# nv-tlabs/NKSR

Hardware: AMD Instinct MI355X
Metric: reconstructed points/sec (solve+mesh) (higher is better)
Workload: dtype f32

## Files before the change

### include/nksr_hip.h

```cpp
#ifndef NKSR_HIP_H
#define NKSR_HIP_H
#include <stddef.h>
#include <stdint.h>

#ifdef __cplusplus
extern "C" {
#endif

#define NKSR_MAX_DEPTH 6
#define NKSR_OK 0
#define NKSR_ERR_ARG (-1)
#define NKSR_ERR_HIP (-2)
#define NKSR_ERR_CAPACITY (-3)

const char* nksr_last_error(void);
int nksr_version(void);

typedef struct {
    int32_t n;
    int32_t offset;
    const int64_t* keys;
    const int32_t* ijk;
    const int32_t* nbr;
    const int64_t* hkeys;
// ... 239 lines not shown
int nksr_edge_seam_flags(const nksr_chunk_grid_t* grid, const int64_t* vkey, const int8_t* axis, int64_t n, int32_t cells_per_voxel, float w0,
                         const int32_t* owner, int32_t rank, uint8_t* flags_out, void* stream);
int nksr_points_owner_flags(const nksr_chunk_grid_t* grid, const float* xyz, int64_t n, float reach, const int32_t* owner, int32_t rank,
                            uint8_t* flags_out, void* stream);
int nksr_halo_band_flags(const int64_t* keys, const int32_t* ijk, int64_t n, const int64_t* klo, int32_t nchunk, const float* shift,
                         const float* tlo, const float* thi, float w, int32_t* seg_out, int32_t* flags_out, void* stream);

int nksr_knn_pca_normals(const float* xyz_sorted, int64_t n, const int32_t* start, const int32_t* end,
                         const int64_t* hkeys, const int32_t* hvals, int32_t hcap, float cell, float inv_cell, int k,
                         int max_ring, float* normal_out, float* radius2_out, int32_t* valid_out,
                         int32_t* todo_work ,
                         void* stream);
#define NKSR_KNN_LEVELS 12
typedef struct {
    const float* xyz_sorted;
    const int32_t* start[NKSR_KNN_LEVELS];
    const int32_t* end[NKSR_KNN_LEVELS];
    const int32_t* child[NKSR_KNN_LEVELS];
    const uint8_t* cmask[NKSR_KNN_LEVELS];
    const int64_t* hkeys[NKSR_KNN_LEVELS];
    const int32_t* hvals[NKSR_KNN_LEVELS];
    int32_t hcap[NKSR_KNN_LEVELS];
    int32_t levels, leaf;
    float cell, inv_cell;
} nksr_knn_pyramid_t;
int nksr_knn_pyramid_level(const int64_t* child_keys, int32_t n_child, const int32_t* child_start, const int32_t* child_end,
                           const int64_t* keys, int32_t n, int32_t* child_out, uint8_t* cmask_out, int32_t* start_out, int32_t* end_out,
                           void* stream);
int nksr_sdf_from_points_pyramid(const nksr_knn_pyramid_t* pyramid, const float* normal_sorted, const float* ref_std_sorted, const float* query,
                                 int64_t nq, int k, int max_ring, float stdv, int imls, float* sdf_out, float* grad_out, int32_t* valid_out,
                                 void* stream);
int nksr_knn_mean_dist_pyramid(const nksr_knn_pyramid_t* pyramid, int64_t n, int k, int max_ring, float* out, int32_t* valid_out, void* stream);
int nksr_sdf_from_points(const float* xyz_sorted, const float* normal_sorted, const float* ref_std_sorted, const int32_t* start,
                         const int32_t* end, const int64_t* hkeys, const int32_t* hvals, int32_t hcap, float cell, float inv_cell,
                         const float* query, int64_t nq, int k, int max_ring, float stdv, int imls, float* sdf_out, float* grad_out,
                         int32_t* valid_out, void* stream);
int nksr_knn_mean_dist(const float* xyz_sorted, int64_t n, const int32_t* start, const int32_t* end, const int64_t* hkeys,
                       const int32_t* hvals, int32_t hcap, float cell, float inv_cell, int k, int max_ring, float* out,
                       int32_t* valid_out, void* stream);
int nksr_nearest_index(const float* xyz_sorted, const int32_t* start, const int32_t* end, const int64_t* hkeys,
                       const int32_t* hvals, int32_t hcap, float cell, float inv_cell, const float* query, int64_t nq,
                       int max_ring, int32_t* index_out, void* stream);
int nksr_knn_query_pyramid(const nksr_knn_pyramid_t* pyramid, int64_t n_ref, const float* query, int64_t nq, int k, int exclude_self,
                           const int32_t* self_index, int max_ring, int32_t* idx_out, float* dist2_out, int32_t* valid_out, void* stream);
int nksr_radius_count(const float* xyz_sorted, int64_t n_ref, const int32_t* start, const int32_t* end, const int64_t* hkeys,
                      const int32_t* hvals, int32_t hcap, float cell, float inv_cell, const float* query, int64_t nq, float radius,
                      int32_t cap, int exclude_self, const int32_t* self_index, int32_t* count_out, void* stream);

#define NKSR_ICP_BLOCK 256
#define NKSR_ICP_FIELDS 32
#define NKSR_ICP_COUNT 0
#define NKSR_ICP_D2 1
#define NKSR_ICP_PT_P 2
#define NKSR_ICP_PT_Q 5
#define NKSR_ICP_PT_PQ 8
#define NKSR_ICP_PL_JJ 2
#define NKSR_ICP_PL_JR 23
#define NKSR_ICP_PL_RR 29
int nksr_icp_accumulate(const float* xyz_sorted, int64_t n_ref, const int32_t* start, const int32_t* end, const int64_t* hkeys,
                        const int32_t* hvals, int32_t hcap, float cell, float inv_cell, const int64_t* perm, const float* normal_sorted,
                        const float* source, int64_t n_src, const double* transform, const double* centre, float radius, int method,
                        int64_t* corr_out, double* partials_out, void* stream);
int nksr_icp_reduce(const double* partials, int64_t nrows, double* sums_out, void* stream);

#define NKSR_VOXEL_REDUCE_MAX_C 16
int nksr_voxel_reduce(const int32_t* order, int64_t n, const int32_t* start, const int32_t* end, int64_t n_vox, const float* xyz,
                      const float* attr, int C, int group, float* mean_xyz_out, float* mean_attr_out, int32_t* count_out,
                      int32_t* nearest_out, void* stream);

int nksr_base_cell_flags(const int32_t* nbr, int32_t n, int32_t* flags, void* stream);
int nksr_base_cell_keys(const int32_t* ijk, const int32_t* sel, int64_t nsel, int upsample, int64_t* cell_keys, void* stream);
int nksr_level_cell_keys(const int32_t* ijk, const int32_t* sel, int64_t nsel, int level, int upsample, int64_t* cell_keys, void* stream);
int nksr_cell_corner_keys(const int64_t* cell_keys, int64_t ncell, int64_t* corner_keys, void* stream);
int nksr_lattice_positions(const int64_t* vkeys, int64_t n, float h, float half_w0, float* xyz_out, void* stream);
int nksr_sorted_lookup(const int64_t* sorted, int64_t n, const int64_t* q, int64_t nq, int32_t* idx_out, void* stream);
int nksr_rank_sorted(const int64_t* sorted, int64_t n, const int64_t* q, int64_t nq, int upper, int32_t* rank_out, void* stream);
int nksr_cell_config(const int32_t* corner_idx, const float* f, int64_t ncell, int32_t* config, int32_t* ntri, void* stream);
int nksr_cell_active_flags(const int32_t* config, int64_t ncell, int32_t* flags, void* stream);
int nksr_compact_block_counts(const int32_t* flags, int64_t n, int32_t* block_counts, void* stream);
int nksr_compact_scatter(const int32_t* flags, int64_t n, const int32_t* block_offsets, int32_t* sel, void* stream);
int nksr_mise_constrain(const int64_t* vkeys_fine, int64_t nv, float* f_fine, const int64_t* chash_keys, const int32_t* chash_vals,
                        int32_t chash_cap, const float* f_coarse, const int64_t* ahash_keys, const int32_t* ahash_vals,
                        int32_t ahash_cap, void* stream);
int nksr_cell_children(const int64_t* cell_keys, const int32_t* sel, int64_t nsel, int64_t* child_keys, void* stream);
int nksr_mc_emit(const int32_t* corner_idx, const int32_t* config, const int32_t* tri_offset, int64_t ncell,
                 int64_t* edge_keys, void* stream);
int nksr_mc_vertices(const int64_t* edge_keys, int64_t nedge, const int64_t* vkeys, const int64_t* vhash_keys, const int32_t* vhash_vals,
                     int32_t vhash_cap, const float* vpos, const float* f, float h, float* verts_out, void* stream);

#define NKSR_CELL_SIZES 12
typedef struct {
    int32_t nlev;
    int32_t lam[NKSR_CELL_SIZES];
    int32_t offset[NKSR_CELL_SIZES];
    int32_t hcap[NKSR_CELL_SIZES];
    const int64_t* hkeys[NKSR_CELL_SIZES];
    const int32_t* hvals[NKSR_CELL_SIZES];
} nksr_cell_table_t;
int nksr_adaptive_corner_keys(const int64_t* cell_keys, int64_t ncell, int lam, int64_t* corner_keys_out, void* stream);
int nksr_adaptive_dual_cells(const int64_t* corner_keys, int64_t ncorner, const nksr_cell_table_t* table, int32_t* cidx_out, void* stream);
int nksr_adaptive_positions(const int64_t* cell_keys, const int32_t* cell_lam, int64_t ncell, float u, float* xyz_out, void* stream);
int nksr_mc_emit_pairs(const int32_t* corner_idx, const int32_t* config, const int32_t* tri_offset, int64_t ncell, int64_t* pair_keys,
                       void* stream);
int nksr_pair_vertices(const int64_t* pair_keys, int64_t npair, const int64_t* cell_keys, const int32_t* cell_lam, const float* cell_pos,
                       const float* f, float u, float* verts_out, void* stream);


int nksr_mesh_face_areas(const float* v, int64_t nv, const void* faces, int faces_int64, int64_t nf, float* normal_out, double* area_out,
                         void* stream);
int nksr_inclusive_sum_f64(void* tmp, size_t* tmp_bytes, const double* in, double* out, int64_t n, void* stream);
int nksr_mesh_sample(const float* v, int64_t nv, const void* faces, int faces_int64, int64_t nf, const double* cdf, const float* face_normal,
                     int64_t n, uint64_t seed, float* xyz_out, float* normal_out, int64_t* face_out, void* stream);
#define NKSR_NN_BLOCK 128
#define NKSR_METRIC_NTHRESH 5
#define NKSR_METRIC_FIELDS 8
#define NKSR_METRIC_THRESHOLDS {0.01, 0.015, 0.02, 0.002, 0.1}
int nksr_nn_metrics(const nksr_knn_pyramid_t* pyramid, const int64_t* top_keys, int32_t n_top, const float* normal_sorted, const float* query,
                    const float* query_normal, int64_t nq, int max_ring, float* dist_out, float* dot_out, double* partials_out, void* stream);
int nksr_metric_reduce(const double* partials, int64_t nrows, double* out, void* stream);

#define NKSR_BVH_NODE_FLOATS 16
#define NKSR_BVH_LEAF_FLOATS 12
#define NKSR_BVH_STACK 64
#define NKSR_BVH_MAX_FACES (1ll << 30)
#define NKSR_BVH_MAX_RAYS 7
#define NKSR_BVH_RAY_DIRS {{0.5f, 0.25f, 1.0f}, {1.0f, -0.375f, 0.625f}, {-0.625f, 1.0f, -0.25f}, {-0.25f, -0.5f, -1.0f}, \
                           {-1.0f, 0.625f, -0.375f}, {0.375f, -1.0f, 0.5f}, {-0.375f, 0.75f, 1.0f}}
typedef struct {
    int64_t n_faces;
    int32_t depth;
    int32_t reserved;
    float* nodes;
    float* leaves;
    const float* box;
    int32_t* depth_dev;
} nksr_bvh_t;
int nksr_bvh_morton(const float* xyz, int64_t nv, const void* faces, int faces_int64, int64_t n, const float* box6, uint64_t* codes_out,
                    uint32_t* index_out, void* stream);
int nksr_bvh_nodes(const uint64_t* codes_sorted, int32_t* parent_work, const nksr_bvh_t* bvh, void* stream);
int nksr_bvh_refit(const float* v, int64_t nv, const void* faces, int faces_int64, const uint32_t* order, const int32_t* parent_work,
                   int32_t* flag_work, const nksr_bvh_t* bvh, void* stream);
int nksr_mesh_occupancy(const nksr_bvh_t* bvh, const float* query, int64_t nq, const uint32_t* order, int rays, uint8_t* inside_out,
                        int32_t* counts_out, void* stream);
int nksr_mesh_closest(const nksr_bvh_t* bvh, const float* query, int64_t nq, const uint32_t* order, float* dist_out, int64_t* face_out,
                      float* point_out, void* stream);

#define NKSR_TOPO_MAX_FACES (1ll << 30)
#define NKSR_TOPO_BOUNDARY 1
#define NKSR_TOPO_INTERIOR 2
#define NKSR_TOPO_MISORIENTED 3
#define NKSR_TOPO_NONMANIFOLD 4
#define NKSR_TOPO_TOTALS 6
int nksr_topo_halfedge_keys(const void* faces, int faces_int64, int64_t nf, int64_t nv, uint64_t* keys_out, uint32_t* ids_out,
                            uint8_t* face_valid_out, uint8_t* vertex_ref_out, void* stream);
int nksr_topo_edge_classes(const void* faces, int faces_int64, int64_t nf, int64_t nv, const uint32_t* ids_sorted, const uint64_t* edge_keys,
                           const uint32_t* edge_start, int64_t n_edges, const uint8_t* vertex_ref, int32_t* edge_v_out, int32_t* edge_count_out,
                           uint8_t* edge_class_out, int32_t* face_adj_out, int64_t* totals_out, void* stream);
int nksr_topo_face_pairs(const uint64_t* keys_sorted, const uint32_t* ids_sorted, int64_t n_half, int64_t nv, int32_t* pairs_out, void* stream);
int nksr_uf_components(int32_t* parent, int64_t n, const uint8_t* valid, const int32_t* pairs, int64_t n_pairs, int32_t* root_flags_out,
                       void* stream);
int nksr_uf_labels(const int32_t* parent, int64_t n, const int32_t* root_rank, int32_t* label_out, void* stream);
int nksr_topo_cross_labels(const void* faces, int faces_int64, int64_t nf, int64_t nv, const uint8_t* face_valid, int from_vertices,
                           int32_t* face_label, int32_t* vertex_label, void* stream);
int nksr_topo_component_counts(const int32_t* face_label, int64_t nf, const int32_t* vertex_label, int64_t nv, const uint32_t* ids_sorted,
                               const uint32_t* edge_start, const uint8_t* edge_class, int64_t n_edges, int64_t n_comp, int64_t* counts_out,
                               void* stream);
int nksr_topo_shared_corners(const void* faces, int faces_int64, int64_t nf, int64_t nv, const int32_t* face_label, const int32_t* vertex_label,
                             uint64_t* keys_out, int64_t capacity, int64_t* count_out, void* stream);
int nksr_topo_count_shared(const uint64_t* keys_sorted, int64_t m, int64_t n_comp, int64_t* counts, void* stream);
int nksr_topo_component_boxes(const float* v, int64_t nv, const void* faces, int faces_int64, int64_t nf, const int32_t* face_label,
                              int64_t n_comp, float* box_out, void* stream);
// ... 124 lines not shown
```

### nksr_amd/csrc/meshing.hip

```cpp
#include "common.h"
#pragma clang fp contract(off)
#include "mc_table.h"

#define CMP_BLOCK 256

__global__ void __launch_bounds__(CMP_BLOCK) k_flag_block_count(const int32_t* __restrict__ flags, int64_t n,
                                                                 int32_t* __restrict__ block_counts) {
    __shared__ int wsum[CMP_BLOCK / 64];
    int64_t i = (int64_t)blockIdx.x * CMP_BLOCK + threadIdx.x;
    bool f = i < n && flags[i] != 0;
    unsigned long long m = __ballot(f);
    if ((threadIdx.x & 63) == 0) wsum[threadIdx.x >> 6] = __popcll(m);
    __syncthreads();
    if (threadIdx.x == 0) {
        int t = 0;
        for (int w = 0; w < CMP_BLOCK / 64; ++w) t += wsum[w];
        block_counts[blockIdx.x] = t;
    }
}

__global__ void __launch_bounds__(CMP_BLOCK) k_flag_block_scatter(const int32_t* __restrict__ flags, int64_t n,
                                                                   const int32_t* __restrict__ block_offsets,
                                                                   int32_t* __restrict__ sel) {
    __shared__ int wsum[CMP_BLOCK / 64];
// ... 68 lines not shown
}

__global__ void k_cell_children(const int64_t* __restrict__ cell_keys, const int32_t* __restrict__ sel, int64_t nsel,
                                int64_t* __restrict__ child) {
    int64_t t = (int64_t)blockIdx.x * blockDim.x + threadIdx.x;
    if (t >= nsel * 8) return;
    int x, y, z;
    morton_decode_biased(cell_keys[sel[t >> 3]], NKSR_BIAS0, x, y, z);
    int c = (int)(t & 7);
    child[t] = morton_biased(2 * x + (c >> 2), 2 * y + ((c >> 1) & 1), 2 * z + (c & 1), NKSR_BIAS0);
}

__global__ void k_lattice_positions(const int64_t* __restrict__ vkeys, int64_t n, float h, float half_w0,
                                    float* __restrict__ xyz) {
    int64_t i = (int64_t)blockIdx.x * blockDim.x + threadIdx.x;
    if (i >= n) return;
    int x, y, z;
    morton_decode_biased(vkeys[i], NKSR_BIAS0, x, y, z);
    const float px = (float)x * h, py = (float)y * h, pz = (float)z * h;
    xyz[i * 3] = px + half_w0;
    xyz[i * 3 + 1] = py + half_w0;
    xyz[i * 3 + 2] = pz + half_w0;
}

__global__ void k_cell_config(const int32_t* __restrict__ corner_idx, const float* __restrict__ f, int64_t ncell,
                              int32_t* __restrict__ config, int32_t* __restrict__ ntri) {
    int64_t i = (int64_t)blockIdx.x * blockDim.x + threadIdx.x;
    if (i >= ncell) return;
    int cfg = 0, j[8], lowest = 0;
#pragma unroll
    for (int c = 0; c < 8; ++c) { j[c] = corner_idx[i * 8 + c]; lowest = j[c] < lowest ? j[c] : lowest; }
#pragma unroll
    for (int c = 0; c < 8; ++c) cfg |= (f[j[c] < 0 ? 0 : j[c]] > 0.f) ? (1 << c) : 0;
    if (lowest < 0) cfg = 0;
    config[i] = cfg;
    ntri[i] = MC_NTRI[cfg];
}

__global__ void k_cell_active_flags(const int32_t* __restrict__ config, int64_t ncell, int32_t* __restrict__ flags) {
    int64_t i = (int64_t)blockIdx.x * blockDim.x + threadIdx.x;
    if (i >= ncell) return;
    int c = config[i];
    flags[i] = (c != 0 && c != 255) ? 1 : 0;
}

__global__ void k_mc_emit(const int32_t* __restrict__ corner_idx, const int32_t* __restrict__ config,
                          const int32_t* __restrict__ tri_offset, int64_t ncell, int64_t* __restrict__ edge_keys) {
    int64_t i = (int64_t)blockIdx.x * blockDim.x + threadIdx.x;
    if (i >= ncell) return;
    const int cfg = config[i];
    const int nt = MC_NTRI[cfg];
    int64_t o = (int64_t)tri_offset[i] * 3;
    for (int t = 0; t < nt * 3; ++t) {
        int e = MC_TRI[cfg][t];
        edge_keys[o + t] = (int64_t)corner_idx[i * 8 + MC_EDGE_LO[e]] * 3 + MC_EDGE_AXIS[e];
    }
}

__global__ void k_mc_vertices(const int64_t* __restrict__ edge_keys, int64_t nedge, const int64_t* __restrict__ vkeys,
                              const int64_t* __restrict__ hkeys, const int32_t* __restrict__ hvals, int hcap,
                              const float* __restrict__ vpos, const float* __restrict__ f, float h,
                              float* __restrict__ verts) {
    int64_t i = (int64_t)blockIdx.x * blockDim.x + threadIdx.x;
    if (i >= nedge) return;
    int64_t ek = edge_keys[i];
    int64_t v0 = ek / 3;
    int axis = (int)(ek % 3);
    int g[3];
    morton_decode_biased(vkeys[v0], NKSR_BIAS0, g[0], g[1], g[2]);
    g[axis] += 1;
    const int64_t k1 = morton_biased(g[0], g[1], g[2], NKSR_BIAS0);
    const int v1 = hash_find(hkeys, hvals, hcap, k1);
    float f0 = f[v0], f1 = f[v1 >= 0 ? v1 : v0];
    const float df = f0 - f1;
    const float t = f0 / df;
    float p[3] = {vpos[v0 * 3], vpos[v0 * 3 + 1], vpos[v0 * 3 + 2]};
    const float th = t * h;
    p[axis] = p[axis] + th;
    verts[i * 3] = p[0];
    verts[i * 3 + 1] = p[1];
    verts[i * 3 + 2] = p[2];
}

#define LAUNCH1D(kern, n, stream, ...)                                                              \
    do {                                                                                            \
        if ((n) > 0) {                                                                              \
            hipLaunchKernelGGL(kern, dim3(nksr_blocks((n), 256)), dim3(256), 0, (hipStream_t)(stream), __VA_ARGS__); \
            NKSR_CHECK_LAUNCH();                                                                    \
        }                                                                                           \
    } while (0)

extern "C" int nksr_base_cell_flags(const int32_t* nbr, int32_t n, int32_t* flags, void* stream) {
    LAUNCH1D(k_base_cell_flags, (int64_t)n, stream, nbr, n, flags);
    return NKSR_OK;
}
extern "C" int nksr_base_cell_keys(const int32_t* ijk, const int32_t* sel, int64_t nsel, int upsample, int64_t* cell_keys, void* stream) {
    if (upsample < 1 || upsample > 8) return nksr_set_error(NKSR_ERR_ARG, "grid_upsample must be in [1,8]");
    LAUNCH1D(k_base_cell_keys, nsel * upsample * upsample * upsample, stream, ijk, sel, nsel, upsample, cell_keys);
    return NKSR_OK;
}
extern "C" int nksr_level_cell_keys(const int32_t* ijk, const int32_t* sel, int64_t nsel, int level, int upsample, int64_t* cell_keys, void* stream) {
    if (upsample < 1 || upsample > 8) return nksr_set_error(NKSR_ERR_ARG, "grid_upsample must be in [1,8]");
    if (level < 0 || level >= NKSR_MAX_DEPTH || (upsample << level) > 64) return nksr_set_error(NKSR_ERR_ARG, "bad level / upsample");
    const int64_t S = (int64_t)upsample << level;
    LAUNCH1D(k_level_cell_keys, nsel * S * S * S, stream, ijk, sel, nsel, level, upsample, cell_keys);
    return NKSR_OK;
}
extern "C" int nksr_cell_corner_keys(const int64_t* cell_keys, int64_t ncell, int64_t* corner_keys, void* stream) {
    LAUNCH1D(k_cell_corner_keys, ncell * 8, stream, cell_keys, ncell, corner_keys);
    return NKSR_OK;
}
extern "C" int nksr_cell_children(const int64_t* cell_keys, const int32_t* sel, int64_t nsel, int64_t* child_keys, void* stream) {
    LAUNCH1D(k_cell_children, nsel * 8, stream, cell_keys, sel, nsel, child_keys);
    return NKSR_OK;
}
extern "C" int nksr_lattice_positions(const int64_t* vkeys, int64_t n, float h, float half_w0, float* xyz_out, void* stream) {
    LAUNCH1D(k_lattice_positions, n, stream, vkeys, n, h, half_w0, xyz_out);
    return NKSR_OK;
}
extern "C" int nksr_cell_config(const int32_t* corner_idx, const float* f, int64_t ncell, int32_t* config, int32_t* ntri, void* stream) {
    LAUNCH1D(k_cell_config, ncell, stream, corner_idx, f, ncell, config, ntri);
    return NKSR_OK;
}
extern "C" int nksr_cell_active_flags(const int32_t* config, int64_t ncell, int32_t* flags, void* stream) {
    LAUNCH1D(k_cell_active_flags, ncell, stream, config, ncell, flags);
    return NKSR_OK;
}
extern "C" int nksr_mc_emit(const int32_t* corner_idx, const int32_t* config, const int32_t* tri_offset, int64_t ncell,
                            int64_t* edge_keys, void* stream) {
    LAUNCH1D(k_mc_emit, ncell, stream, corner_idx, config, tri_offset, ncell, edge_keys);
    return NKSR_OK;
}
extern "C" int nksr_mc_vertices(const int64_t* edge_keys, int64_t nedge, const int64_t* vkeys, const int64_t* vhash_keys,
                                const int32_t* vhash_vals, int32_t vhash_cap, const float* vpos, const float* f, float h, float* verts_out,
                                void* stream) {
    LAUNCH1D(k_mc_vertices, nedge, stream, edge_keys, nedge, vkeys, vhash_keys, vhash_vals, vhash_cap, vpos, f, h, verts_out);
    return NKSR_OK;
}

__global__ void k_mise_constrain(const int64_t* __restrict__ vkeys_fine, int64_t nv, float* __restrict__ f_fine,
                                 const int64_t* __restrict__ ch_keys, const int32_t* __restrict__ ch_vals, int ch_cap,
                                 const float* __restrict__ f_coarse, const int64_t* __restrict__ ah_keys,
                                 const int32_t* __restrict__ ah_vals, int ah_cap) {
    int64_t i = (int64_t)blockIdx.x * blockDim.x + threadIdx.x;
    if (i >= nv) return;
    int g[3];
    morton_decode_biased(vkeys_fine[i], NKSR_BIAS0, g[0], g[1], g[2]);
    const int odd[3] = {g[0] & 1, g[1] & 1, g[2] & 1};
    const int k = odd[0] + odd[1] + odd[2];
    if (k == 3) return;
    if (k == 0) {
        const int j = hash_find(ch_keys, ch_vals, ch_cap, morton_biased(g[0] >> 1, g[1] >> 1, g[2] >> 1, NKSR_BIAS0));
        if (j >= 0) f_fine[i] = f_coarse[j];
        return;
    }
    int lo[3], cnt[3];
#pragma unroll
    for (int a = 0; a < 3; ++a) {
        lo[a] = odd[a] ? (g[a] - 1) >> 1 : (g[a] >> 1) - 1;
        cnt[a] = odd[a] ? 1 : 2;
    }
    bool all_active = true;
    for (int x = 0; x < cnt[0]; ++x)
        for (int y = 0; y < cnt[1]; ++y)
            for (int z = 0; z < cnt[2]; ++z)
                all_active = all_active && hash_find(ah_keys, ah_vals, ah_cap, morton_biased(lo[0] + x, lo[1] + y, lo[2] + z, NKSR_BIAS0)) >= 0;
    if (all_active) return;
    float s = 0.f;
    int n = 0;
    for (int x = 0; x <= odd[0]; ++x)
        for (int y = 0; y <= odd[1]; ++y)
            for (int z = 0; z <= odd[2]; ++z) {
                const int cx = odd[0] ? ((g[0] - 1) >> 1) + x : g[0] >> 1, cy = odd[1] ? ((g[1] - 1) >> 1) + y : g[1] >> 1,
                          cz = odd[2] ? ((g[2] - 1) >> 1) + z : g[2] >> 1;
                const int j = hash_find(ch_keys, ch_vals, ch_cap, morton_biased(cx, cy, cz, NKSR_BIAS0));
                if (j >= 0) { s += f_coarse[j]; ++n; }
            }
    if (n == (1 << k)) f_fine[i] = s * (k == 1 ? 0.5f : 0.25f);
}

extern "C" int nksr_mise_constrain(const int64_t* vkeys_fine, int64_t nv, float* f_fine, const int64_t* chash_keys, const int32_t* chash_vals,
                                   int32_t chash_cap, const float* f_coarse, const int64_t* ahash_keys, const int32_t* ahash_vals,
                                   int32_t ahash_cap, void* stream) {
    LAUNCH1D(k_mise_constrain, nv, stream, vkeys_fine, nv, f_fine, chash_keys, chash_vals, chash_cap, f_coarse, ahash_keys, ahash_vals, ahash_cap);
    return NKSR_OK;
}

__global__ void k_adaptive_corner_keys(const int64_t* __restrict__ cell_keys, int64_t ncell, int lam, int64_t* __restrict__ out) {
    int64_t t = (int64_t)blockIdx.x * blockDim.x + threadIdx.x;
    if (t >= ncell * 8) return;
    int x, y, z;
    morton_decode_biased(cell_keys[t >> 3], NKSR_BIAS0, x, y, z);
    const int c = (int)(t & 7), s = 1 << lam;
    out[t] = morton_biased((x + (c >> 2)) * s - 1, (y + ((c >> 1) & 1)) * s - 1, (z + (c & 1)) * s - 1, NKSR_BIAS0);
}

__global__ void k_adaptive_dual_cells(const int64_t* __restrict__ corner_keys, int64_t ncorner, nksr_cell_table_t T,
                                      int32_t* __restrict__ cidx) {
    int64_t t = (int64_t)blockIdx.x * blockDim.x + threadIdx.x;
    if (t >= ncorner * 8) return;
    int x, y, z;
    morton_decode_biased(corner_keys[t >> 3], NKSR_BIAS0, x, y, z);
    const int c = (int)(t & 7);
    x += c >> 2; y += (c >> 1) & 1; z += c & 1;
    int id = -1;
    for (int l = 0; l < T.nlev; ++l) {
        if (id >= 0) continue;
        const int sh = T.lam[l];
        const int j = hash_find(T.hkeys[l], T.hvals[l], T.hcap[l], morton_biased(x >> sh, y >> sh, z >> sh, NKSR_BIAS0));
        if (j >= 0) id = T.offset[l] + j;
    }
    cidx[t] = id;
}

__global__ void k_adaptive_positions(const int64_t* __restrict__ cell_keys, const int32_t* __restrict__ cell_lam, int64_t n, float u,
                                     float* __restrict__ xyz) {
    int64_t i = (int64_t)blockIdx.x * blockDim.x + threadIdx.x;
    if (i >= n) return;
    int x, y, z;
    morton_decode_biased(cell_keys[i], NKSR_BIAS0, x, y, z);
    const int s = 1 << cell_lam[i];
    const float half = (float)s * (0.5f * u);
    const float px = (float)(x * s) * u, py = (float)(y * s) * u, pz = (float)(z * s) * u;
    xyz[i * 3] = px + half;
    xyz[i * 3 + 1] = py + half;
    xyz[i * 3 + 2] = pz + half;
}

__global__ void k_mc_emit_pairs(const int32_t* __restrict__ corner_idx, const int32_t* __restrict__ config,
                                const int32_t* __restrict__ tri_offset, int64_t ncell, int64_t* __restrict__ pair_keys) {
    int64_t i = (int64_t)blockIdx.x * blockDim.x + threadIdx.x;
    if (i >= ncell) return;
    const int cfg = config[i];
    const int nt = MC_NTRI[cfg];
    int64_t o = (int64_t)tri_offset[i] * 3;
    for (int t = 0; t < nt * 3; ++t) {
        const int e = MC_TRI[cfg][t];
        const int lo = MC_EDGE_LO[e], axis = MC_EDGE_AXIS[e];
        const int64_t a = corner_idx[i * 8 + lo], b = corner_idx[i * 8 + (lo | (4 >> axis))];
        pair_keys[o + t] = (a << 33) | ((int64_t)axis << 31) | b;
    }
}

__global__ void k_pair_vertices(const int64_t* __restrict__ pair_keys, int64_t npair, const int64_t* __restrict__ cell_keys,
                                const int32_t* __restrict__ cell_lam, const float* __restrict__ cell_pos, const float* __restrict__ f,
                                float u, float* __restrict__ verts) {
    int64_t i = (int64_t)blockIdx.x * blockDim.x + threadIdx.x;
    if (i >= npair) return;
    const int64_t k = pair_keys[i];
    const int64_t a = k >> 33, b = k & 0x7FFFFFFFll;
    int ca[3], cb[3];
    morton_decode_biased(cell_keys[a], NKSR_BIAS0, ca[0], ca[1], ca[2]);
    morton_decode_biased(cell_keys[b], NKSR_BIAS0, cb[0], cb[1], cb[2]);
    const int sa = 1 << cell_lam[a], sb = 1 << cell_lam[b];
    const float fa = f[a], fb = f[b];
    const float t = fa / (fa - fb);
    const float hu = 0.5f * u;
#pragma unroll
    for (int x = 0; x < 3; ++x) {
        const int d2 = 2 * (cb[x] * sb - ca[x] * sa) + (sb - sa);
        const float d = (float)d2 * hu;
// ... 34 lines not shown
```

### nksr_amd/meshing.py

```python
import os

import torch

from . import ops
from ._lib import call, ptr, stream
from .fields.base_field import MeshingResult


def _cell_vertices(cell_keys_raw):
    dev = cell_keys_raw.device
    cells = ops.sort_unique(cell_keys_raw, maybe_sorted=True)
    nc = cells.numel()
    ck = torch.empty(nc * 8, dtype=torch.int64, device=dev)
    call('nksr_cell_corner_keys', ptr(cells), nc, ptr(ck), stream())
    vkeys = ops.sort_unique(ops.dedup_corner_keys(cells) if nc >= (1 << 16) else ck)
    vhash = ops.HashTable(vkeys)
    cidx = vhash.query(ck).view(nc, 8)
    return cells, vkeys, cidx, vhash


def extract_dual_mesh(field, mise_iter=0, grid_upsample=1, max_points=-1):
    spread = hasattr(field, 'finalize_mesh') and (getattr(field, 'world_size', 1) > 1 or getattr(field, 'distributed', False))
    if getattr(field, 'dual_graph', 'lattice') == 'adaptive':
        if not spread:
            return _extract_adaptive(field, mise_iter, grid_upsample, max_points)
        from . import chunking
        need = chunking.halo_inner(field.svh.voxel_size, getattr(field, 'meshing_depth', 1), 'adaptive')
        if getattr(field, 'world_size', 1) > 1 and (getattr(field, 'halo_inner', None) is None or field.halo_inner < need - 1e-6 * need):
            raise RuntimeError("dual_graph='adaptive' on a chunked field spread over several ranks needs halos %.3g deep (set "
                               "Reconstructor.dual_graph = 'adaptive' BEFORE reconstruct(); this field's are %s)"
                               % (need, getattr(field, 'halo_inner', None)))
        return field.finalize_mesh_named(_extract_adaptive(field, mise_iter, grid_upsample, max_points, owned=True))
    res = _extract(field, mise_iter, grid_upsample, max_points)
    if hasattr(field, 'finalize_mesh'):
        res = field.finalize_mesh(res)
    return res


def _extract(field, mise_iter, grid_upsample, max_points):
    svh = field.svh
    dev = svh.device
    g0 = svh.level(0)
    w0 = svh.voxel_size
    U = int(grid_upsample)
    empty = MeshingResult(torch.zeros((0, 3), dtype=torch.float32, device=dev), torch.zeros((0, 3), dtype=torch.int64, device=dev))
    empty.edge_vkey = torch.zeros(0, dtype=torch.int64, device=dev)
    empty.edge_axis = torch.zeros(0, dtype=torch.int8, device=dev)
    batch = max_points if (max_points is not None and max_points > 0) else (1 << 22)
    if U < 1 or mise_iter < 0:
        raise RuntimeError('grid_upsample must be >= 1 and mise_iter >= 0')
    owned_only = hasattr(field, 'base_cell_mask') and getattr(field, 'world_size', 1) > 1
    use_seam = owned_only and dev.type == 'cuda' and hasattr(field, 'seam_flags') and os.environ.get('NKSR_SEAM_FLAGS', '1') != '0'
    if use_seam:
        empty.seam_flag = torch.zeros(0, dtype=torch.uint8, device=dev)
    adaptive = max(1, min(int(getattr(field, 'meshing_depth', 1)), svh.depth))
    levels = [d for d in range(adaptive) if svh.level(d).num_voxels > 0]
    if not levels:
        return empty
    reach = max(((int(svh.level(d).ijk.abs().max()) + 4) << d) for d in levels) * U * (1 << int(mise_iter)) + 2
    if reach >= (1 << 20):
        raise RuntimeError('mesh lattice out of range: |ijk| * grid_upsample * 2^mise_iter = %d >= 2^20; recentre the cloud '
                           '(or lower mise_iter / grid_upsample)' % reach)

    raw = torch.empty(0, dtype=torch.int64, device=dev)
    if g0.num_voxels:
        flags = torch.empty(g0.num_voxels, dtype=torch.int32, device=dev)
        call('nksr_base_cell_flags', ptr(g0.nbr), g0.num_voxels, ptr(flags), stream())
        if owned_only:
            flags = (flags * field.base_cell_halo_mask(g0.ijk).to(torch.int32)).contiguous()
        sel = ops.compact(flags)
        raw = torch.empty(sel.numel() * U ** 3, dtype=torch.int64, device=dev)
        if sel.numel():
            call('nksr_base_cell_keys', ptr(g0.ijk), ptr(sel), sel.numel(), U, ptr(raw), stream())
    for d in levels:
        if d == 0:
            continue
        gd = svh.level(d)
        fl = torch.empty(gd.num_voxels, dtype=torch.int32, device=dev)
        call('nksr_base_cell_flags', ptr(gd.nbr), gd.num_voxels, ptr(fl), stream())
        sd = ops.compact(fl)
        if sd.numel():
            S = U << d
            rd = torch.empty(sd.numel() * S ** 3, dtype=torch.int64, device=dev)
            call('nksr_level_cell_keys', ptr(gd.ijk), ptr(sd), sd.numel(), d, U, ptr(rd), stream())
            if owned_only:
                gc = torch.empty((rd.numel(), 3), dtype=torch.int32, device=dev)
                call('nksr_decode_keys', ptr(rd), rd.numel(), -1, ptr(gc), stream())
                rd = rd[field.base_cell_halo_mask(torch.div(gc, U, rounding_mode='floor').to(torch.int32))]
            raw = torch.cat([raw, rd])
    if raw.numel() == 0:
        return empty

    h = w0 / U
    prev = None
    for m in range(mise_iter + 1):
        cells, vkeys, cidx, vhash = _cell_vertices(raw)
        nv, nc = vkeys.numel(), cells.numel()
        pos = torch.empty((nv, 3), dtype=torch.float32, device=dev)
        call('nksr_lattice_positions', ptr(vkeys), nv, float(h), float(0.5 * w0), ptr(pos), stream())
        f = field._evaluate_f_model(pos, False, max_points=batch).value
        if prev is not None:
            ch, ah = prev[0], prev[2]
            call('nksr_mise_constrain', ptr(vkeys), nv, ptr(f), ptr(ch.hkeys), ptr(ch.hvals), ch.cap, ptr(prev[1]), ptr(ah.hkeys), ptr(ah.hvals),
                 ah.cap, stream())
        config = torch.empty(nc, dtype=torch.int32, device=dev)
        ntri = torch.empty(nc + 1, dtype=torch.int32, device=dev)
        ntri[nc] = 0
        call('nksr_cell_config', ptr(cidx), ptr(f), nc, ptr(config), ptr(ntri), stream())
        if m < mise_iter:
            act = torch.empty(nc, dtype=torch.int32, device=dev)
            call('nksr_cell_active_flags', ptr(config), nc, ptr(act), stream())
            asel = ops.compact(act)
            if asel.numel() == 0:
                return empty
            raw = torch.empty(asel.numel() * 8, dtype=torch.int64, device=dev)
            call('nksr_cell_children', ptr(cells), ptr(asel), asel.numel(), ptr(raw), stream())
            prev = (vhash, f, ops.HashTable(cells[asel.long()].contiguous()))
            h = h / 2

    if owned_only:
        gc = torch.empty((nc, 3), dtype=torch.int32, device=dev)
        call('nksr_decode_keys', ptr(cells), nc, -1, ptr(gc), stream())
        base_ijk = torch.div(gc, U * (1 << mise_iter), rounding_mode='floor').to(torch.int32)
        keep_c = field.base_cell_mask(base_ijk).to(torch.int32)
        ntri[:nc] *= keep_c
        config = (config * keep_c).contiguous()
    tri_off = ops.exclusive_sum_i32(ntri)
    T = int(tri_off[nc].item())
    if T == 0:
        return empty
    ekeys = torch.empty(T * 3, dtype=torch.int64, device=dev)
    call('nksr_mc_emit', ptr(cidx), ptr(config), ptr(tri_off), nc, ptr(ekeys), stream())
    uek = ops.sort_unique(ops.dedup_keys(ekeys) if ekeys.numel() >= (1 << 19) else ekeys)
    faces = ops.HashTable(uek).query(ekeys).view(T, 3)
    ne = uek.numel()
    verts = torch.empty((ne, 3), dtype=torch.float32, device=dev)
    call('nksr_mc_vertices', ptr(uek), ne, ptr(vkeys), ptr(vhash.hkeys), ptr(vhash.hvals), vhash.cap, ptr(pos), ptr(f), float(h), ptr(verts), stream())

    ev = torch.div(uek, 3, rounding_mode='floor')
    edge_vkey, edge_axis = vkeys[ev], (uek - ev * 3).to(torch.int8)
    verts, faces, (edge_vkey, edge_axis) = _trim(field, verts, faces, (edge_vkey, edge_axis), masked=True)
    res = _result(field, verts, faces)
    res.edge_vkey, res.edge_axis, res.lattice_h = edge_vkey, edge_axis, h
    if use_seam:
        res.seam_flag = field.seam_flags(edge_vkey, edge_axis, U * (1 << mise_iter))
    return res


def _trim(field, verts, faces, per_vertex=(), masked=True, drop_unused=False):
    dev = verts.device
    ne = verts.shape[0]
    keep_v = field.mask_vertices(verts) if masked else None
    trimmed = keep_v is not None and not bool(keep_v.all())
    if trimmed:
        faces = faces[keep_v[faces.long()].all(1)]
    if trimmed or drop_unused:
        used = torch.zeros(ne, dtype=torch.int32, device=dev)
        used[faces.reshape(-1).long()] = 1
        remap = ops.exclusive_sum_i32(used)
        vsel = ops.compact(used).long()
        verts = verts[vsel]
        per_vertex = tuple(a[vsel] for a in per_vertex)
        faces = remap[faces.long()]
    return verts, faces, per_vertex


def _result(field, verts, faces):
    v_world = verts / field.scale if field.scale != 1.0 else verts
    colors = None
    if field.texture_field is not None:
        colors = field.texture_field.evaluate_color(v_world)
    return MeshingResult(v_world, faces.long(), colors)


def _leaf_coordinates(svh, adaptive):
    dev = svh.device
    out = [[] for _ in range(adaptive)]
    for d in range(adaptive):
        g = svh.level(d)
        if g.num_voxels == 0:
            continue
        if d == 0:
            out[0].append(g.ijk)
            continue
        child = svh.level(d - 1)
        internal = torch.zeros(g.num_voxels, dtype=torch.bool, device=dev)
        if child.num_voxels:
            pi = g.hash.query((child.keys >> 3).contiguous())
            internal[pi[pi >= 0].long()] = True
        out[d].append(g.ijk[~internal])
        ik = g.keys[internal]
        if ik.numel():
            ck = ((ik[:, None] << 3) | torch.arange(8, dtype=torch.int64, device=dev)[None]).reshape(-1).contiguous()
            vk = ck[child.hash.query(ck) < 0].contiguous()
            if vk.numel():
                vijk = torch.empty((vk.numel(), 3), dtype=torch.int32, device=dev)
                call('nksr_decode_keys', ptr(vk), vk.numel(), d - 1, ptr(vijk), stream())
                out[d - 1].append(vijk)
    return [torch.cat(o) if o else torch.zeros((0, 3), dtype=torch.int32, device=dev) for o in out]


class _CellTable:

    def __init__(self, pieces, dev):
        from ._lib import CELL_SIZES, CellTableT
        self.lams = sorted(l for l in pieces if sum(p[0].numel() for p in pieces[l]))
        if len(self.lams) > CELL_SIZES:
            raise RuntimeError('adaptive dual graph: more than %d cell sizes' % CELL_SIZES)
        self.keys, self.hashes, self.offset = {}, {}, {}
        t = CellTableT()
        n, fs, ks, ls = 0, [], [], []
        self.all_new = all(p[1] is None for l in self.lams for p in pieces[l] if p[0].numel())
        self.any_new = any(p[1] is None for l in self.lams for p in pieces[l] if p[0].numel())
        nan = float('nan')
        for i, l in enumerate(self.lams):
            ps = [p for p in pieces[l] if p[0].numel()]
            if len(ps) == 1:
                ko = ps[0][0].contiguous()
                f = ps[0][1] if ps[0][1] is not None else (None if self.all_new else torch.full((ko.numel(),), nan, dtype=torch.float32, device=dev))
            else:
                k = torch.cat([p[0] for p in ps])
                ko, order = ops.sort_pairs(k, torch.arange(k.numel(), dtype=torch.int32, device=dev))
                f = None
# ... 154 lines not shown
```

Before: 31.47 million.

## Skip field evaluation for MISE-constrained vertices and dedup MC edges via slot marking

During MISE refinement, vertices whose value is fully determined by the coarse level are now filled directly, and only the remaining vertices are compacted, gathered and passed to the expensive field evaluation, then scattered back. Marching-cubes edge deduplication no longer emits per-triangle edge keys and sorts/hashes them. Instead it marks used edge slots in a dense 3*nv array, prefix-sums that array to get edge ids, and writes faces and vertices directly. This removes sort and hash costs and most of the redundant network evaluation. In exchange it adds extra kernels and a dense slot array sized to the lattice, plus a host sync to read the edge count.

```diff
diff --git a/include/nksr_hip.h b/include/nksr_hip.h
--- a/include/nksr_hip.h
+++ b/include/nksr_hip.h
@@ -345,11 +345,22 @@
 int nksr_mise_constrain(const int64_t* vkeys_fine, int64_t nv, float* f_fine, const int64_t* chash_keys, const int32_t* chash_vals,
                         int32_t chash_cap, const float* f_coarse, const int64_t* ahash_keys, const int32_t* ahash_vals,
                         int32_t ahash_cap, void* stream);
+int nksr_mise_constrain_first(const int64_t* vkeys_fine, int64_t nv, float* f_fine, const int64_t* chash_keys, const int32_t* chash_vals,
+                              int32_t chash_cap, const float* f_coarse, const int64_t* ahash_keys, const int32_t* ahash_vals,
+                              int32_t ahash_cap, int32_t* flag_out, void* stream);
+int nksr_gather_rows3_f32(const float* src, const int32_t* sel, int64_t nsel, float* dst, void* stream);
+int nksr_scatter_f32(const float* src, const int32_t* sel, int64_t nsel, float* dst, void* stream);
 int nksr_cell_children(const int64_t* cell_keys, const int32_t* sel, int64_t nsel, int64_t* child_keys, void* stream);
 int nksr_mc_emit(const int32_t* corner_idx, const int32_t* config, const int32_t* tri_offset, int64_t ncell,
                  int64_t* edge_keys, void* stream);
 int nksr_mc_vertices(const int64_t* edge_keys, int64_t nedge, const int64_t* vkeys, const int64_t* vhash_keys, const int32_t* vhash_vals,
                      int32_t vhash_cap, const float* vpos, const float* f, float h, float* verts_out, void* stream);
+int nksr_mc_mark_edges(const int32_t* corner_idx, const int32_t* config, int64_t ncell, int32_t* used, int32_t* far_out, void* stream);
+int nksr_mc_faces(const int32_t* corner_idx, const int32_t* config, const int32_t* tri_offset, int64_t ncell, const int32_t* eid,
+                  int32_t* faces_out, void* stream);
+int nksr_mc_edge_vertices(const int32_t* used, const int32_t* eid, const int32_t* far_in, int64_t nslot, const int64_t* vkeys,
+                          const float* vpos, const float* f, float h, float* verts_out, int64_t* edge_vkey_out, int8_t* edge_axis_out,
+                          void* stream);
 
 #define NKSR_CELL_SIZES 12
 typedef struct {
diff --git a/nksr_amd/csrc/meshing.hip b/nksr_amd/csrc/meshing.hip
--- a/nksr_amd/csrc/meshing.hip
+++ b/nksr_amd/csrc/meshing.hip
@@ -174,6 +174,73 @@
     verts[i * 3 + 2] = p[2];
 }
 
+__global__ void k_mc_mark_edges(const int32_t* __restrict__ corner_idx, const int32_t* __restrict__ config, int64_t ncell,
+                                int32_t* __restrict__ used, int32_t* __restrict__ far) {
+    int64_t i = (int64_t)blockIdx.x * blockDim.x + threadIdx.x;
+    if (i >= ncell) return;
+    const int cfg = config[i];
+    const int nt = MC_NTRI[cfg];
+    int mask = 0;
+    for (int t = 0; t < nt * 3; ++t) mask |= 1 << MC_TRI[cfg][t];
+    for (int e = 0; e < 12; ++e) {
+        if (!((mask >> e) & 1)) continue;
+        const int lo = MC_EDGE_LO[e], axis = MC_EDGE_AXIS[e];
+        const int64_t p = (int64_t)corner_idx[i * 8 + lo] * 3 + axis;
+        used[p] = 1;
+        far[p] = corner_idx[i * 8 + (lo | (4 >> axis))];
+    }
+}
+
+__global__ void k_mc_faces(const int32_t* __restrict__ corner_idx, const int32_t* __restrict__ config,
+                           const int32_t* __restrict__ tri_offset, int64_t ncell, const int32_t* __restrict__ eid,
+                           int32_t* __restrict__ faces) {
+    int64_t i = (int64_t)blockIdx.x * blockDim.x + threadIdx.x;
+    if (i >= ncell) return;
+    const int cfg = config[i];
+    const int nt = MC_NTRI[cfg];
+    int64_t o = (int64_t)tri_offset[i] * 3;
+    for (int t = 0; t < nt * 3; ++t) {
+        int e = MC_TRI[cfg][t];
+        faces[o + t] = eid[(int64_t)corner_idx[i * 8 + MC_EDGE_LO[e]] * 3 + MC_EDGE_AXIS[e]];
+    }
+}
+
+__global__ void k_mc_edge_vertices(const int32_t* __restrict__ used, const int32_t* __restrict__ eid, const int32_t* __restrict__ far,
+                                   int64_t nslot, const int64_t* __restrict__ vkeys, const float* __restrict__ vpos,
+                                   const float* __restrict__ f, float h, float* __restrict__ verts, int64_t* __restrict__ edge_vkey,
+                                   int8_t* __restrict__ edge_axis) {
+    int64_t p = (int64_t)blockIdx.x * blockDim.x + threadIdx.x;
+    if (p >= nslot || !used[p]) return;
+    const int64_t i = eid[p];
+    int64_t v0 = p / 3;
+    int axis = (int)(p % 3);
+    const int v1 = far[p];
+    float f0 = f[v0], f1 = f[v1 >= 0 ? v1 : v0];
+    const float df = f0 - f1;
+    const float t = f0 / df;
+    float q[3] = {vpos[v0 * 3], vpos[v0 * 3 + 1], vpos[v0 * 3 + 2]};
+    const float th = t * h;
+    q[axis] = q[axis] + th;
+    verts[i * 3] = q[0];
+    verts[i * 3 + 1] = q[1];
+    verts[i * 3 + 2] = q[2];
+    edge_vkey[i] = vkeys[v0];
+    edge_axis[i] = (int8_t)axis;
+}
+
+__global__ void k_gather_rows3(const float* __restrict__ src, const int32_t* __restrict__ sel, int64_t nsel, float* __restrict__ dst) {
+    int64_t t = (int64_t)blockIdx.x * blockDim.x + threadIdx.x;
+    if (t >= nsel * 3) return;
+    const int64_t r = t / 3;
+    dst[t] = src[(int64_t)sel[r] * 3 + (t - r * 3)];
+}
+
+__global__ void k_scatter_f32(const float* __restrict__ src, const int32_t* __restrict__ sel, int64_t nsel, float* __restrict__ dst) {
+    int64_t i = (int64_t)blockIdx.x * blockDim.x + threadIdx.x;
+    if (i >= nsel) return;
+    dst[sel[i]] = src[i];
+}
+
 #define LAUNCH1D(kern, n, stream, ...)                                                              \
     do {                                                                                            \
         if ((n) > 0) {                                                                              \
@@ -229,22 +296,44 @@
     LAUNCH1D(k_mc_vertices, nedge, stream, edge_keys, nedge, vkeys, vhash_keys, vhash_vals, vhash_cap, vpos, f, h, verts_out);
     return NKSR_OK;
 }
-
-__global__ void k_mise_constrain(const int64_t* __restrict__ vkeys_fine, int64_t nv, float* __restrict__ f_fine,
-                                 const int64_t* __restrict__ ch_keys, const int32_t* __restrict__ ch_vals, int ch_cap,
-                                 const float* __restrict__ f_coarse, const int64_t* __restrict__ ah_keys,
-                                 const int32_t* __restrict__ ah_vals, int ah_cap) {
-    int64_t i = (int64_t)blockIdx.x * blockDim.x + threadIdx.x;
-    if (i >= nv) return;
+extern "C" int nksr_mc_mark_edges(const int32_t* corner_idx, const int32_t* config, int64_t ncell, int32_t* used, int32_t* far_out,
+                                  void* stream) {
+    LAUNCH1D(k_mc_mark_edges, ncell, stream, corner_idx, config, ncell, used, far_out);
+    return NKSR_OK;
+}
+extern "C" int nksr_mc_faces(const int32_t* corner_idx, const int32_t* config, const int32_t* tri_offset, int64_t ncell, const int32_t* eid,
+                             int32_t* faces_out, void* stream) {
+    LAUNCH1D(k_mc_faces, ncell, stream, corner_idx, config, tri_offset, ncell, eid, faces_out);
+    return NKSR_OK;
+}
+extern "C" int nksr_mc_edge_vertices(const int32_t* used, const int32_t* eid, const int32_t* far_in, int64_t nslot, const int64_t* vkeys,
+                                     const float* vpos, const float* f, float h, float* verts_out, int64_t* edge_vkey_out,
+                                     int8_t* edge_axis_out, void* stream) {
+    if (nslot >= (1ll << 31)) return nksr_set_error(NKSR_ERR_ARG, "edge slots: 3 nv must stay below 2^31");
+    LAUNCH1D(k_mc_edge_vertices, nslot, stream, used, eid, far_in, nslot, vkeys, vpos, f, h, verts_out, edge_vkey_out, edge_axis_out);
+    return NKSR_OK;
+}
+extern "C" int nksr_gather_rows3_f32(const float* src, const int32_t* sel, int64_t nsel, float* dst, void* stream) {
+    LAUNCH1D(k_gather_rows3, nsel * 3, stream, src, sel, nsel, dst);
+    return NKSR_OK;
+}
+extern "C" int nksr_scatter_f32(const float* src, const int32_t* sel, int64_t nsel, float* dst, void* stream) {
+    LAUNCH1D(k_scatter_f32, nsel, stream, src, sel, nsel, dst);
+    return NKSR_OK;
+}
+
+__device__ __forceinline__ bool mise_replacement(int64_t vkey_fine, const int64_t* __restrict__ ch_keys, const int32_t* __restrict__ ch_vals,
+                                                 int ch_cap, const float* __restrict__ f_coarse, const int64_t* __restrict__ ah_keys,
+                                                 const int32_t* __restrict__ ah_vals, int ah_cap, float& out) {
     int g[3];
-    morton_decode_biased(vkeys_fine[i], NKSR_BIAS0, g[0], g[1], g[2]);
+    morton_decode_biased(vkey_fine, NKSR_BIAS0, g[0], g[1], g[2]);
     const int odd[3] = {g[0] & 1, g[1] & 1, g[2] & 1};
     const int k = odd[0] + odd[1] + odd[2];
-    if (k == 3) return;
+    if (k == 3) return false;
     if (k == 0) {
         const int j = hash_find(ch_keys, ch_vals, ch_cap, morton_biased(g[0] >> 1, g[1] >> 1, g[2] >> 1, NKSR_BIAS0));
-        if (j >= 0) f_fine[i] = f_coarse[j];
-        return;
+        if (j >= 0) out = f_coarse[j];
+        return j >= 0;
     }
     int lo[3], cnt[3];
 #pragma unroll
@@ -257,7 +346,7 @@
         for (int y = 0; y < cnt[1]; ++y)
             for (int z = 0; z < cnt[2]; ++z)
                 all_active = all_active && hash_find(ah_keys, ah_vals, ah_cap, morton_biased(lo[0] + x, lo[1] + y, lo[2] + z, NKSR_BIAS0)) >= 0;
-    if (all_active) return;
+    if (all_active) return false;
     float s = 0.f;
     int n = 0;
     for (int x = 0; x <= odd[0]; ++x)
@@ -268,7 +357,38 @@
                 const int j = hash_find(ch_keys, ch_vals, ch_cap, morton_biased(cx, cy, cz, NKSR_BIAS0));
                 if (j >= 0) { s += f_coarse[j]; ++n; }
             }
-    if (n == (1 << k)) f_fine[i] = s * (k == 1 ? 0.5f : 0.25f);
+    if (n == (1 << k)) out = s * (k == 1 ? 0.5f : 0.25f);
+    return n == (1 << k);
+}
+
+__global__ void k_mise_constrain(const int64_t* __restrict__ vkeys_fine, int64_t nv, float* __restrict__ f_fine,
+                                 const int64_t* __restrict__ ch_keys, const int32_t* __restrict__ ch_vals, int ch_cap,
+                                 const float* __restrict__ f_coarse, const int64_t* __restrict__ ah_keys,
+                                 const int32_t* __restrict__ ah_vals, int ah_cap) {
+    int64_t i = (int64_t)blockIdx.x * blockDim.x + threadIdx.x;
+    if (i >= nv) return;
+    float v;
+    if (mise_replacement(vkeys_fine[i], ch_keys, ch_vals, ch_cap, f_coarse, ah_keys, ah_vals, ah_cap, v)) f_fine[i] = v;
+}
+
+__global__ void k_mise_constrain_first(const int64_t* __restrict__ vkeys_fine, int64_t nv, float* __restrict__ f_fine,
+                                       const int64_t* __restrict__ ch_keys, const int32_t* __restrict__ ch_vals, int ch_cap,
+                                       const float* __restrict__ f_coarse, const int64_t* __restrict__ ah_keys,
+                                       const int32_t* __restrict__ ah_vals, int ah_cap, int32_t* __restrict__ flag) {
+    int64_t i = (int64_t)blockIdx.x * blockDim.x + threadIdx.x;
+    if (i >= nv) return;
+    float v;
+    const bool replaced = mise_replacement(vkeys_fine[i], ch_keys, ch_vals, ch_cap, f_coarse, ah_keys, ah_vals, ah_cap, v);
+    if (replaced) f_fine[i] = v;
+    flag[i] = replaced ? 0 : 1;
+}
+
+extern "C" int nksr_mise_constrain_first(const int64_t* vkeys_fine, int64_t nv, float* f_fine, const int64_t* chash_keys,
+                                         const int32_t* chash_vals, int32_t chash_cap, const float* f_coarse, const int64_t* ahash_keys,
+                                         const int32_t* ahash_vals, int32_t ahash_cap, int32_t* flag_out, void* stream) {
+    LAUNCH1D(k_mise_constrain_first, nv, stream, vkeys_fine, nv, f_fine, chash_keys, chash_vals, chash_cap, f_coarse, ahash_keys, ahash_vals,
+             ahash_cap, flag_out);
+    return NKSR_OK;
 }
 
 extern "C" int nksr_mise_constrain(const int64_t* vkeys_fine, int64_t nv, float* f_fine, const int64_t* chash_keys, const int32_t* chash_vals,
diff --git a/nksr_amd/meshing.py b/nksr_amd/meshing.py
--- a/nksr_amd/meshing.py
+++ b/nksr_amd/meshing.py
@@ -98,11 +98,20 @@
         nv, nc = vkeys.numel(), cells.numel()
         pos = torch.empty((nv, 3), dtype=torch.float32, device=dev)
         call('nksr_lattice_positions', ptr(vkeys), nv, float(h), float(0.5 * w0), ptr(pos), stream())
-        f = field._evaluate_f_model(pos, False, max_points=batch).value
-        if prev is not None:
+        if prev is None:
+            f = field._evaluate_f_model(pos, False, max_points=batch).value
+        else:
             ch, ah = prev[0], prev[2]
-            call('nksr_mise_constrain', ptr(vkeys), nv, ptr(f), ptr(ch.hkeys), ptr(ch.hvals), ch.cap, ptr(prev[1]), ptr(ah.hkeys), ptr(ah.hvals),
-                 ah.cap, stream())
+            f = torch.empty(nv, dtype=torch.float32, device=dev)
+            need = torch.empty(nv, dtype=torch.int32, device=dev)
+            call('nksr_mise_constrain_first', ptr(vkeys), nv, ptr(f), ptr(ch.hkeys), ptr(ch.hvals), ch.cap, ptr(prev[1]), ptr(ah.hkeys),
+                 ptr(ah.hvals), ah.cap, ptr(need), stream())
+            sel = ops.compact(need)
+            if sel.numel():
+                ps = torch.empty((sel.numel(), 3), dtype=torch.float32, device=dev)
+                call('nksr_gather_rows3_f32', ptr(pos), ptr(sel), sel.numel(), ptr(ps), stream())
+                fs = field._evaluate_f_model(ps, False, max_points=batch).value.contiguous()
+                call('nksr_scatter_f32', ptr(fs), ptr(sel), sel.numel(), ptr(f), stream())
         config = torch.empty(nc, dtype=torch.int32, device=dev)
         ntri = torch.empty(nc + 1, dtype=torch.int32, device=dev)
         ntri[nc] = 0
@@ -129,16 +138,21 @@
     T = int(tri_off[nc].item())
     if T == 0:
         return empty
-    ekeys = torch.empty(T * 3, dtype=torch.int64, device=dev)
-    call('nksr_mc_emit', ptr(cidx), ptr(config), ptr(tri_off), nc, ptr(ekeys), stream())
-    uek = ops.sort_unique(ops.dedup_keys(ekeys) if ekeys.numel() >= (1 << 19) else ekeys)
-    faces = ops.HashTable(uek).query(ekeys).view(T, 3)
-    ne = uek.numel()
+    ns = 3 * nv
+    if ns >= (1 << 31) - 1:
+        raise RuntimeError('mesh lattice too large: %d vertices (3 per vertex edge slots must stay below 2^31)' % nv)
+    used = torch.zeros(ns + 1, dtype=torch.int32, device=dev)
+    far = torch.empty(ns, dtype=torch.int32, device=dev)
+    call('nksr_mc_mark_edges', ptr(cidx), ptr(config), nc, ptr(used), ptr(far), stream())
+    eid = ops.exclusive_sum_i32(used)
+    ne = int(eid[ns].item())
+    faces = torch.empty((T, 3), dtype=torch.int32, device=dev)
+    call('nksr_mc_faces', ptr(cidx), ptr(config), ptr(tri_off), nc, ptr(eid), ptr(faces), stream())
     verts = torch.empty((ne, 3), dtype=torch.float32, device=dev)
-    call('nksr_mc_vertices', ptr(uek), ne, ptr(vkeys), ptr(vhash.hkeys), ptr(vhash.hvals), vhash.cap, ptr(pos), ptr(f), float(h), ptr(verts), stream())
-
-    ev = torch.div(uek, 3, rounding_mode='floor')
-    edge_vkey, edge_axis = vkeys[ev], (uek - ev * 3).to(torch.int8)
+    edge_vkey = torch.empty(ne, dtype=torch.int64, device=dev)
+    edge_axis = torch.empty(ne, dtype=torch.int8, device=dev)
+    call('nksr_mc_edge_vertices', ptr(used), ptr(eid), ptr(far), ns, ptr(vkeys), ptr(pos), ptr(f), float(h), ptr(verts), ptr(edge_vkey),
+         ptr(edge_axis), stream())
     verts, faces, (edge_vkey, edge_axis) = _trim(field, verts, faces, (edge_vkey, edge_axis), masked=True)
     res = _result(field, verts, faces)
     res.edge_vkey, res.edge_axis, res.lattice_h = edge_vkey, edge_axis, h
```

Result: faster. 32.18 million (median of 6 runs) (+2.2%).
